# minjiyoon/MMGL

Hardware: AMD Instinct MI355X
Metric: train samples/sec (OPT-1.3B flamingo, 16 neighbors) (higher is better)
Workload: dtype bf16; 1 GPU; opt-1.3b context=all neighbor_mode=embedding peft=flamingo, 11+5 neighbors x 4 tokens, T=512+128, roberta-base + clip-vit-base-patch16 frozen encoders, full train step (fwd+bwd+exchange+AdamW); per_gpu_batch=64, global_batch=64, seq_len=640, neighbor_keys=64, trainable_params=216736520, parallelism=dp1

## Files before the change

include/mmgl_hip.h:

```cpp
#ifndef MMGL_HIP_H
#define MMGL_HIP_H

#include <stddef.h>
#include <stdint.h>

#ifdef __cplusplus
extern "C" {
#endif

enum { MMGL_F32 = 0, MMGL_BF16 = 1 };
enum { MMGL_OK = 0, MMGL_ERR_INVALID = 1, MMGL_ERR_UNSUPPORTED = 2, MMGL_ERR_HIP = 3 };
enum { MMGL_ACT_NONE = 0, MMGL_ACT_RELU = 1 };

const char* mmgl_last_error(void);
int mmgl_version(void);

int mmgl_xattn_fwd(const void* q, const void* k, const void* v, const uint8_t* key_valid,
                   void* out, float* lse, int B, int H, int T, int S, int D, int dtype, void* stream);

size_t mmgl_xattn_bwd_workspace(int B, int H, int T, int S, int D);
int mmgl_xattn_bwd(const void* dout, const void* q, const void* k, const void* v, const float* lse,
                   const uint8_t* key_valid, void* dq, void* dk, void* dv,
                   void* workspace, size_t workspace_bytes,
                   int B, int H, int T, int S, int D, int dtype, void* stream);
// ... 51 lines not shown
size_t mmgl_norm_bwd_workspace(int rows, int cols);
int mmgl_layernorm_bwd(const void* dy, const void* x, const void* gamma, const float* mean, const float* rstd,
                       void* dx, float* dgamma, float* dbeta, void* workspace, size_t workspace_bytes,
                       int rows, int cols, int dtype, void* stream);

int mmgl_rmsnorm_fwd(const void* x, const void* gamma, void* y, float* rstd,
                     int rows, int cols, float eps, int dtype, void* stream);
int mmgl_rmsnorm_bwd(const void* dy, const void* x, const void* gamma, const float* rstd,
                     void* dx, float* dgamma, void* workspace, size_t workspace_bytes,
                     int rows, int cols, int dtype, void* stream);

int mmgl_add_rmsnorm_fwd(const void* x, const void* res, const void* gamma, void* sum_out, void* y, float* rstd,
                         int rows, int cols, float eps, int dtype, void* stream);
int mmgl_add_rmsnorm_bwd(const void* dy, const void* dsum, const void* sum, const void* gamma, const float* rstd,
                         void* dres, float* dgamma, void* workspace, size_t workspace_bytes,
                         int rows, int cols, int dtype, void* stream);

int mmgl_gated_residual_fwd(const void* residual, const void* x, const float* gate, void* y,
                            size_t n, float p_drop, uint64_t seed, int dtype, void* stream);
size_t mmgl_gated_residual_bwd_workspace(size_t n);
int mmgl_gated_residual_bwd(const void* dy, const void* x, const float* gate, void* dx, float* dgate,
                            void* workspace, size_t workspace_bytes,
                            size_t n, float p_drop, uint64_t seed, int dtype, void* stream);

int mmgl_linear_fwd(const void* x, const void* W, const void* bias, void* y,
                    int M, int N, int K, int act, float out_scale, int dtype, void* stream);
size_t mmgl_linear_bwd_workspace(int M, int N, int K, int act, int dtype);
int mmgl_linear_bwd(const void* dy, const void* y, const void* x, const void* W, void* dx, void* dW, void* dbias,
                    void* workspace, size_t workspace_bytes, int M, int N, int K, int act, float out_scale,
                    int accumulate, int mask_dx, int dtype, void* stream);

int mmgl_lora_linear_fwd(const void* x, const void* W, const void* bias, const void* A, const void* Bm,
                         void* y, void* xa, int M, int N, int K, int r, float scale, int dtype, void* stream);
size_t mmgl_lora_linear_bwd_workspace(int M, int N, int K, int r, int dtype);
int mmgl_lora_linear_bwd(const void* dy, const void* x, const void* xa, const void* W, const void* A,
                         const void* Bm, void* dx, void* dA, void* dB, void* dyb, void* workspace,
                         size_t workspace_bytes, int M, int N, int K, int r, float scale, int accumulate,
                         int dtype, void* stream);

int mmgl_neighbor_interleave_fwd(const void* text_emb, const void* vis_emb, const int64_t* text_loc,
                                 const int64_t* img_loc, const int64_t* text_pos, const int64_t* img_pos,
                                 void* out_emb, uint8_t* out_valid, int B, int Nt, int Ni, int n_tok, int d,
                                 int dtype, void* stream);
int mmgl_neighbor_interleave_bwd(const void* d_out_emb, const int64_t* text_loc, const int64_t* img_loc,
                                 void* d_text_emb, void* d_vis_emb, int B, int Nt, int Ni, int n_tok, int d,
                                 int dtype, void* stream);

int mmgl_cross_entropy_fwd(const void* logits, const int64_t* labels, float* row_lse, float* row_loss,
                           float* loss_sum, float* count, int rows, int V, int64_t ignore_index, int dtype,
                           void* stream);
int mmgl_cross_entropy_bwd(const void* logits, const int64_t* labels, const float* row_lse,
                           const float* count, const float* dloss, void* dlogits,
                           int rows, int V, int64_t ignore_index, int dtype, void* stream);

int mmgl_position_ids(const int64_t* attention_mask, int64_t* pos, int B, int T, void* stream);

int mmgl_adamw_step(void* param, float* master, const void* grad, float* exp_avg, float* exp_avg_sq, size_t n,
                    float lr, float beta1, float beta2, float eps, float weight_decay, int step,
                    float grad_scale, int dtype, void* stream);

size_t mmgl_adafactor_workspace(const int64_t* segs, int n, int64_t* table_out);
int mmgl_adafactor_step(void* param, float* master, const void* grad, float* state, const int64_t* table, const int64_t* table_host,
                        int n, void* workspace, size_t workspace_bytes, float lr, float eps1, float clip_threshold, double decay_rate,
                        float weight_decay, int step, float grad_scale, int dtype, void* stream);

int mmgl_gemm_nt_fast(int M, int N, int K, int ldx, int ldw, int ldy, int dtype);
size_t mmgl_gemm_nt_workspace(int M, int N, int K, int ldx, int ldw, int ldy, int dtype);
int mmgl_gemm_nt(const void* x, int ldx, const void* W, int ldw, const void* bias, const void* residual, const void* zmask,
                 void* y, int ldy, int M, int N, int K, int act, float out_scale, void* workspace, size_t workspace_bytes,
                 int dtype, void* stream);
int mmgl_relu_bwd(const void* dy, const void* y, void* out, size_t n, int dtype, void* stream);
int mmgl_gemm_nt_rowk(const void* x, int ldx, const void* W, int ldw, void* y, int ldy, int M, int N, int K, int K_short,
                      int m_full, int dtype, void* stream);
int mmgl_gemm_nt_rowk_item(int G, int n_long, int n_short, int q, int wg, int it);
int mmgl_gemm_set_tile_counter(void* counter);
void* mmgl_gemm_get_tile_counter(void);
size_t mmgl_gemm_nt_relu_bits_bytes(int M, int N, int K, int ldx, int ldw, int ldy, int dtype);
int mmgl_gemm_nt_relu_bits(const void* x, int ldx, const void* W, int ldw, const void* bias, void* y, int ldy, void* bits_out,
                           int M, int N, int K, float out_scale, int dtype, void* stream);
int mmgl_gemm_nt_masked(const void* x, int ldx, const void* W, int ldw, const void* bits_in, void* y, int ldy, int M, int N, int K,
                        float out_scale, int dtype, void* stream);

int mmgl_rope_inplace(void* buf, const float* cos_sin, size_t rows, int T, int H, int D, int ld, int nblk, int backward,
                      int dtype, void* stream);
int mmgl_rope(const void* src, void* dst, const float* cos_sin, size_t rows, int T, int H, int D, int ld, int nblk, int nall,
              int backward, int dtype, void* stream);
int mmgl_swiglu_fwd(const void* gate_up, void* y, size_t M, int F, int dtype, void* stream);
int mmgl_swiglu_bwd(const void* dy, const void* gate_up, void* dgate_up, size_t M, int F, int dtype, void* stream);

int mmgl_encattn_fwd(const void* q, const void* k, const void* v, const int32_t* cu_seqlens, void* out, int nseq,
                     int H, int D, int ld_in, int ld_out, int max_len, int q_rows, int dtype, void* stream);
int mmgl_add_layernorm_fwd(const void* x, const void* res, const void* gamma, const void* beta, void* sum_out,
                           void* y, float* mean, float* rstd, int rows, int cols, float eps, float p_drop, uint64_t seed,
                           int dtype, void* stream);
int mmgl_add_layernorm_bwd(const void* dy, const void* dsum, const void* sum, const void* gamma, const float* mean,
                           const float* rstd, void* dres, void* dx, float* dgamma, float* dbeta, void* workspace,
                           size_t workspace_bytes, int rows, int cols, float p_drop, uint64_t seed, int dtype,
                           void* stream);
int mmgl_layernorm_tiles_fwd(const void* x, const void* gamma, const void* beta, void* y, void* yc, const int32_t* rowmap,
                             float* mean, float* rstd, int rows, int cols, int crows, float eps, int dtype, void* stream);
int mmgl_add_layernorm_tiles_fwd(const void* x, const void* res, const void* gamma, const void* beta, void* sum_out, void* y,
                                 void* yc, const int32_t* rowmap, float* mean, float* rstd, int rows, int cols, int crows,
                                 float eps, float p_drop, uint64_t seed, int dtype, void* stream);
int mmgl_add_layernorm_rows_bwd(const void* dy, const int32_t* dy_rows, const void* dsum, const void* sum, const void* gamma,
                                const float* mean, const float* rstd, void* dres, void* dx, float* dgamma, float* dbeta,
                                void* workspace, size_t workspace_bytes, int rows, int cols, float p_drop, uint64_t seed,
// ... 95 lines not shown
```

mmgl_amd/_lib.py:

```python
import ctypes
import os

import torch

_HERE = os.path.dirname(os.path.abspath(__file__))
LIB_PATH = os.environ.get("MMGL_LIB_PATH") or os.path.join(_HERE, "libmmgl_hip.so")

ABI_VERSION = 110
F32, BF16 = 0, 1
ACT_NONE, ACT_RELU = 0, 1
_ERR_INVALID, _ERR_UNSUPPORTED, _ERR_HIP = 1, 2, 3

c_void_p, c_int, c_float, c_size_t, c_u64, c_i64 = (ctypes.c_void_p, ctypes.c_int, ctypes.c_float, ctypes.c_size_t,
                                                    ctypes.c_uint64, ctypes.c_int64)
P, I, F, Z, U, L = c_void_p, c_int, c_float, c_size_t, c_u64, c_i64
D = ctypes.c_double

SIGNATURES = {
    "mmgl_last_error": (ctypes.c_char_p, []),
    "mmgl_version": (I, []),
    "mmgl_xattn_fwd": (I, [P, P, P, P, P, P, I, I, I, I, I, I, P]),
    "mmgl_xattn_bwd_workspace": (Z, [I, I, I, I, I]),
    "mmgl_xattn_bwd": (I, [P, P, P, P, P, P, P, P, P, P, Z, I, I, I, I, I, I, P]),
    "mmgl_selfattn_fwd": (I, [P, P, P, P, P, P, I, I, I, I, I, I, P]),
    "mmgl_selfattn_bwd_workspace": (Z, [I, I, I]),
    "mmgl_selfattn_bwd": (I, [P, P, P, P, P, P, P, P, P, P, P, Z, I, I, I, I, I, I, I, P]),
    "mmgl_selfattn_prefix_fwd": (I, [P, P, P, P, P, P, I, I, I, I, I, I, I, I, P]),
    "mmgl_selfattn_prefix_bwd": (I, [P, P, P, P, P, P, P, P, P, P, P, Z, I, I, I, I, I, I, I, I, I, I, P]),
    "mmgl_selfattn_tiles_fwd": (I, [P, P, P, P, P, P, P, I, I, I, I, I, I, I, I, P]),
    "mmgl_selfattn_tiles_bwd": (I, [P, P, P, P, P, P, P, P, P, P, P, P, Z, I, I, I, I, I, I, I, I, I, I, P]),
    "mmgl_selfattn_tiles_rows_bwd": (I, [P, P, P, P, P, P, P, P, P, P, P, P, P, Z, I, I, I, I, I, I, I, I, I, I, I, P]),
    "mmgl_selfattn_gqa_fwd": (I, [P, P, P, P, P, P, I, I, I, I, I, I, I, I, P]),
    "mmgl_selfattn_gqa_bwd_workspace": (Z, [I, I, I, I, I, I]),
    "mmgl_selfattn_gqa_bwd": (I, [P, P, P, P, P, P, P, P, P, P, P, Z, I, I, I, I, I, I, I, I, I, I, P]),
    "mmgl_attn_general_fwd": (I, [P, P, P, P, P, P, P, P, I, I, I, I, I, I, F, U, I, P]),
    "mmgl_attn_general_bwd_workspace": (Z, [I, I, I]),
    "mmgl_attn_general_bwd": (I, [P, P, P, P, P, P, P, P, P, P, P, Z, I, I, I, I, I, I, F, U, I, P]),
    "mmgl_attn_dropout_mask": (I, [P, I, I, I, I, F, U, P]),
    "mmgl_attn_relbias_fwd": (I, [P, P, P, P, P, P, P, P, I, I, I, I, I, I, I, I, I, F, U, I, P]),
    "mmgl_attn_relbias_bwd_workspace": (Z, [I, I, I, I]),
    "mmgl_attn_relbias_bwd": (I, [P, P, P, P, P, P, P, P, P, P, P, P, P, P, Z, I, I, I, I, I, I, I, I, I, F, U, I, P]),
    "mmgl_layernorm_fwd": (I, [P, P, P, P, P, P, I, I, F, I, P]),
    "mmgl_norm_bwd_workspace": (Z, [I, I]),
    "mmgl_layernorm_bwd": (I, [P, P, P, P, P, P, P, P, P, Z, I, I, I, P]),
    "mmgl_rmsnorm_fwd": (I, [P, P, P, P, I, I, F, I, P]),
    "mmgl_rmsnorm_bwd": (I, [P, P, P, P, P, P, P, Z, I, I, I, P]),
    "mmgl_add_rmsnorm_fwd": (I, [P, P, P, P, P, P, I, I, F, I, P]),
    "mmgl_add_rmsnorm_bwd": (I, [P, P, P, P, P, P, P, P, Z, I, I, I, P]),
    "mmgl_gated_residual_fwd": (I, [P, P, P, P, Z, F, U, I, P]),
    "mmgl_gated_residual_bwd_workspace": (Z, [Z]),
    "mmgl_gated_residual_bwd": (I, [P, P, P, P, P, P, Z, Z, F, U, I, P]),
    "mmgl_linear_fwd": (I, [P, P, P, P, I, I, I, I, F, I, P]),
    "mmgl_linear_bwd_workspace": (Z, [I, I, I, I, I]),
    "mmgl_linear_bwd": (I, [P, P, P, P, P, P, P, P, Z, I, I, I, I, F, I, I, I, P]),
    "mmgl_lora_linear_fwd": (I, [P, P, P, P, P, P, P, I, I, I, I, F, I, P]),
    "mmgl_lora_linear_bwd_workspace": (Z, [I, I, I, I, I]),
    "mmgl_lora_linear_bwd": (I, [P, P, P, P, P, P, P, P, P, P, P, Z, I, I, I, I, F, I, I, P]),
    "mmgl_neighbor_interleave_fwd": (I, [P, P, P, P, P, P, P, P, I, I, I, I, I, I, P]),
    "mmgl_neighbor_interleave_bwd": (I, [P, P, P, P, P, I, I, I, I, I, I, P]),
    "mmgl_cross_entropy_fwd": (I, [P, P, P, P, P, P, I, I, L, I, P]),
    "mmgl_cross_entropy_bwd": (I, [P, P, P, P, P, P, I, I, L, I, P]),
    "mmgl_position_ids": (I, [P, P, I, I, P]),
    "mmgl_adamw_step": (I, [P, P, P, P, P, Z, F, F, F, F, F, I, F, I, P]),
    "mmgl_encattn_fwd": (I, [P, P, P, P, P, I, I, I, I, I, I, I, I, P]),
    "mmgl_add_layernorm_fwd": (I, [P, P, P, P, P, P, P, P, I, I, F, F, U, I, P]),
    "mmgl_add_layernorm_bwd": (I, [P, P, P, P, P, P, P, P, P, P, P, Z, I, I, F, U, I, P]),
    "mmgl_layernorm_tiles_fwd": (I, [P, P, P, P, P, P, P, P, I, I, I, F, I, P]),
    "mmgl_add_layernorm_tiles_fwd": (I, [P, P, P, P, P, P, P, P, P, P, I, I, I, F, F, U, I, P]),
    "mmgl_activation_fwd": (I, [P, P, Z, I, I, P]),
    "mmgl_scale": (I, [P, P, P, Z, I, P]),
    "mmgl_gemm_nt_fast": (I, [I, I, I, I, I, I, I]),
    "mmgl_gemm_nt_workspace": (Z, [I, I, I, I, I, I, I]),
    "mmgl_gemm_nt_relu_bits_bytes": (Z, [I, I, I, I, I, I, I]),
    "mmgl_gemm_nt_relu_bits": (I, [P, I, P, I, P, P, I, P, I, I, I, F, I, P]),
    "mmgl_gemm_nt_masked": (I, [P, I, P, I, P, P, I, I, I, I, F, I, P]),
    "mmgl_gemm_nt": (I, [P, I, P, I, P, P, P, P, I, I, I, I, I, F, P, Z, I, P]),
    "mmgl_gemm_nt_rowk": (I, [P, I, P, I, P, I, I, I, I, I, I, I, P]),
    "mmgl_gemm_nt_rowk_item": (I, [I, I, I, I, I, I]),
    "mmgl_add_layernorm_rows_bwd": (I, [P, P, P, P, P, P, P, P, P, P, P, P, Z, I, I, F, U, I, P]),
    "mmgl_relu_bwd": (I, [P, P, P, Z, I, P]),
    "mmgl_gemm_set_tile_counter": (I, [P]),
    "mmgl_gemm_get_tile_counter": (P, []),
    "mmgl_rope_inplace": (I, [P, P, Z, I, I, I, I, I, I, I, P]),
    "mmgl_rope": (I, [P, P, P, Z, I, I, I, I, I, I, I, I, P]),
    "mmgl_swiglu_fwd": (I, [P, P, Z, I, I, P]),
    "mmgl_swiglu_bwd": (I, [P, P, P, Z, I, I, P]),
    "mmgl_comm_unique_id": (I, [P]),
    "mmgl_comm_init": (I, [I, I, P, ctypes.POINTER(ctypes.c_void_p)]),
    "mmgl_allreduce_sum": (I, [P, P, Z, I, P]),
    "mmgl_allgather": (I, [P, P, P, Z, I, P]),
    "mmgl_broadcast": (I, [P, P, Z, I, I, P]),
    "mmgl_comm_destroy": (I, [P]),
    "mmgl_gemm_skinny": (I, [P, I, P, I, P, P, P, I, I, I, I, I, F, I, P]),
    "mmgl_attn_decode_fwd": (I, [P, I, P, P, I, Z, P, I, P, I, I, I, I, I, P]),
    "mmgl_gemm_skinny_lora": (I, [P, I, P, I, P, P, P, I, P, I, P, I, I, F, P, I, I, I, I, F, I, P]),
    "mmgl_attn_decode_gqa_fwd": (I, [P, I, P, P, I, Z, P, I, P, I, I, I, I, I, I, P]),
    "mmgl_rope_kv_append": (I, [P, I, P, P, Z, I, I, I, I, I, P]),
    "mmgl_attn_decode_beam_fwd": (I, [P, I, P, P, I, Z, P, I, P, P, I, Z, P, I, P, I, I, I, I, I, I, I, P]),
    "mmgl_beam_topk_workspace": (Z, [I, I, I]),
    "mmgl_beam_topk": (I, [P, Z, P, P, P, P, Z, I, I, I, I, I, P]),
    "mmgl_beam_advance": (I, [P, P, P, P, P, P, P, I, P, P, P, P, P, P, P, P, P, I, I, I, I, I, I, I, F, P]),
    "mmgl_sample_tokens": (I, [P, Z, P, P, L, P, P, I, I, I, F, I, F, I, L, I, P]),
    "mmgl_logits_process": (I, [P, Z, P, Z, P, Z, I, I, P, I, I, I, F, I, I, P]),
    "mmgl_guidance_logits": (I, [P, Z, I, I, F, I, P]),
    "mmgl_attn_decode_block_fwd": (I, [P, I, P, P, I, P, P, I, Z, I, P, I, P, P, I, I, I, I, I, P]),
    "mmgl_lookup_accept": (I, [P, Z, I, P, P, P, P, Z, P, Z, P, P, P, P, I, I, I, I, I, I, L, L, I, I, I, P]),
    "mmgl_rope_kv_append_block": (I, [P, I, P, I, P, I, Z, I, P, I, I, I, I, I, I, P]),
    "mmgl_attn_decode_gqa_block_fwd": (I, [P, I, P, P, I, Z, I, P, I, P, P, I, I, I, I, I, I, P]),
    "mmgl_contrastive_chunk": (I, []),
    "mmgl_contrastive_workspace": (Z, [I, I, I]),
    "mmgl_contrastive_select": (I, [P, Z, P, Z, Z, P, Z, I, P, P, Z, F, I, I, P, Z, P, Z, P, L, L, P, P, P, P, P, P, Z, I, I, I, I, I, P]),
    "mmgl_kv_quantize": (I, [P, P, I, Z, P, I, Z, P, I, Z, I, I, I, I, I, P]),
    "mmgl_attn_decode_q8_fwd": (I, [P, I, P, P, I, P, P, I, Z, P, P, I, Z, I, P, I, P, I, I, I, I, I, P]),
    "mmgl_attn_decode_gqa_q8_fwd": (I, [P, I, P, P, I, P, P, I, Z, P, P, I, Z, I, P, I, P, I, I, I, I, I, I, P]),
# ... 45 lines not shown


def ptr(t):
    return None if t is None else ctypes.c_void_p(t.data_ptr())


def ptr_off(t, nbytes):
    return ctypes.c_void_p(t.data_ptr() + int(nbytes))


_raw_stream = getattr(torch._C, "_cuda_getCurrentRawStream", None)
_raw_device = getattr(torch._C, "_cuda_getDevice", None)


def stream_ptr():
    if _raw_stream is not None and _raw_device is not None:
        return ctypes.c_void_p(_raw_stream(_raw_device()))
    return ctypes.c_void_p(torch.cuda.current_stream().cuda_stream)


def require_cuda(*ts):
    for t in ts:
        if t is not None and not t.is_cuda:
            raise RuntimeError("mmgl_amd ops run on the GPU only (tensor is on %s); there is no CPU path" % t.device)


class KernelTimer:
    enabled = False
    only = None
    records = []
    by_tag = bool(os.environ.get("MMGL_KERNEL_TAGS"))

    @classmethod
    def reset(cls):
        cls.records = []

    @classmethod
    def summary(cls):
        torch.cuda.synchronize()
        out = {}
        for name, s, e, work in cls.records:
            if cls.by_tag and "tag" in work:
                name = f"{name}[{work['tag']}]"
            d = out.setdefault(name, dict(calls=0, ms_total=0.0, bytes=0.0, flops=0.0))
            d["calls"] += 1
            d["ms_total"] += s.elapsed_time(e)
            d["bytes"] += work.get("bytes", 0.0)
            d["flops"] += work.get("flops", 0.0)
        for d in out.values():
            d["ms_avg"] = d["ms_total"] / d["calls"]
        return out


def call(name: str, work, *args):
    fn = getattr(lib(), name)
    if KernelTimer.enabled and (KernelTimer.only is None or name in KernelTimer.only):
        s = torch.cuda.Event(enable_timing=True)
        e = torch.cuda.Event(enable_timing=True)
        s.record()
        rc = fn(*args)
        e.record()
        KernelTimer.records.append((name, s, e, work() if callable(work) else (work or {})))
    else:
        rc = fn(*args)
    check(rc, name)
```

mmgl_amd/csrc/elementwise.hip:

```cpp
#include "common.h"

namespace {

template <typename T> struct Vec {
    static constexpr int N = 16 / sizeof(T);
    typedef T type __attribute__((ext_vector_type(16 / sizeof(T))));
};

__device__ __forceinline__ float block_sum(float v, float* red) {
    v = wave_sum(v);
    __syncthreads();
    if ((threadIdx.x & 63) == 0) red[threadIdx.x >> 6] = v;
    __syncthreads();
    return red[0] + red[1] + red[2] + red[3];
}
__device__ __forceinline__ float block_max(float v, float* red) {
    v = wave_max(v);
    __syncthreads();
    if ((threadIdx.x & 63) == 0) red[threadIdx.x >> 6] = v;
    __syncthreads();
    return fmaxf(fmaxf(red[0], red[1]), fmaxf(red[2], red[3]));
}

inline int stream_blocks(size_t nvec) {
// ... 211 lines not shown

__global__ __launch_bounds__(256) void ce_finish_kernel(const float* __restrict__ row_loss, const int64_t* __restrict__ labels,
                                                        int rows, int V_, int64_t ignore, float* __restrict__ loss_sum,
                                                        float* __restrict__ count) {
    __shared__ float red[4];
    float a = 0.f, c = 0.f;
    for (int i = threadIdx.x; i < rows; i += 256) {
        const int64_t lab = labels[i];
        if (!(lab == ignore || lab < 0 || lab >= V_)) { a += row_loss[i]; c += 1.f; }
    }
    const float sa = block_sum(a, red);
    const float sc = block_sum(c, red);
    if (threadIdx.x == 0) { *loss_sum = sa; *count = sc; }
}

template <typename T>
__global__ __launch_bounds__(256) void ce_bwd_kernel(const T* __restrict__ logits, const int64_t* __restrict__ labels,
                                                     const float* __restrict__ row_lse, const float* __restrict__ count,
                                                     const float* __restrict__ dloss, T* __restrict__ dlogits, int V_,
                                                     int64_t ignore) {
    typedef typename Vec<T>::type V;
    constexpr int VN = Vec<T>::N;
    const int row = blockIdx.x;
    const T* x = logits + (size_t)row * V_;
    T* dx = dlogits + (size_t)row * V_;
    const int64_t lab = labels[row];
    const bool ign = (lab == ignore || lab < 0 || lab >= V_);
    const float scale = ign ? 0.f : (*dloss) / fmaxf(*count, 1.f);
    const float lse = row_lse[row];
    const int nvec = (((size_t)V_ * sizeof(T)) % 16 == 0) ? V_ / VN : 0;
    auto grad = [&](int i, const V& v) __attribute__((always_inline)) {
        V o;
#pragma unroll
        for (int j = 0; j < VN; ++j) {
            float g = __expf((float)v[j] - lse);
            if (i * VN + j == lab) g -= 1.f;
            o[j] = (T)(g * scale);
        }
        ((V*)dx)[i] = o;
    };
    int i = threadIdx.x;
    for (; i + 768 < nvec; i += 1024) {
        const V v0 = ((const V*)x)[i], v1 = ((const V*)x)[i + 256], v2 = ((const V*)x)[i + 512], v3 = ((const V*)x)[i + 768];
        grad(i, v0);
        grad(i + 256, v1);
        grad(i + 512, v2);
        grad(i + 768, v3);
    }
    for (; i < nvec; i += 256) grad(i, ((const V*)x)[i]);
    for (int i = nvec * VN + threadIdx.x; i < V_; i += 256) {
        float g = __expf((float)x[i] - lse);
        if (i == lab) g -= 1.f;
        dx[i] = (T)(g * scale);
    }
}

__global__ __launch_bounds__(64) void position_ids_kernel(const int64_t* __restrict__ mask, int64_t* __restrict__ pos, int T_) {
    const int b = blockIdx.x, lane = threadIdx.x;
    int64_t carry = 0;
    for (int t0 = 0; t0 < T_; t0 += 64) {
        const int t = t0 + lane;
        const int64_t m = t < T_ ? mask[(size_t)b * T_ + t] : 0;
        int64_t v = m;
#pragma unroll
        for (int o = 1; o < 64; o <<= 1) {
            const int64_t u = __shfl_up(v, o);
            if (lane >= o) v += u;
        }
        if (t < T_) pos[(size_t)b * T_ + t] = (carry + v) * m - 1 + 2;
        carry += __shfl(v, 63);
    }
}

template <typename T>
__global__ __launch_bounds__(256) void adamw_kernel(T* __restrict__ param, float* __restrict__ master,
                                                    const T* __restrict__ grad, float* __restrict__ m,
                                                    float* __restrict__ v, size_t n, float lr, float b1, float b2,
                                                    float eps, float wd, float bc1, float bc2s, float gscale) {
    for (size_t i = (size_t)blockIdx.x * 256 + threadIdx.x; i < n; i += (size_t)gridDim.x * 256) {
        const float g = (float)grad[i] * gscale;
        float p = master ? master[i] : (float)param[i];
        p *= 1.f - lr * wd;
        const float mi = b1 * m[i] + (1.f - b1) * g;
        const float vi = b2 * v[i] + (1.f - b2) * g * g;
        m[i] = mi;
        v[i] = vi;
        p -= (lr / bc1) * mi / (sqrtf(vi) / bc2s + eps);
        if (master) master[i] = p;
        param[i] = (T)p;
    }
}

}

#define BY_DTYPE(CALL_BF16, CALL_F32, who)                        \
    do {                                                          \
        if (dtype == MMGL_BF16) { CALL_BF16; }                    \
        else if (dtype == MMGL_F32) { CALL_F32; }                 \
        else MMGL_FAIL(MMGL_ERR_INVALID, "%s: bad dtype %d", who, dtype); \
    } while (0)

extern "C" int mmgl_gated_residual_fwd(const void* residual, const void* x, const float* gate, void* y, size_t n,
                                       float p_drop, uint64_t seed, int dtype, void* stream) {
    MMGL_CHECK_ARG(residual && x && y, "mmgl_gated_residual_fwd: null pointer");
    MMGL_CHECK_ARG(p_drop >= 0.f && p_drop < 1.f, "mmgl_gated_residual_fwd: dropout p=%g outside [0,1)", p_drop);
    if (n == 0) return MMGL_OK;
// ... 55 lines not shown
}

extern "C" int mmgl_neighbor_interleave_bwd(const void* d_out_emb, const int64_t* text_loc, const int64_t* img_loc,
                                            void* d_text_emb, void* d_vis_emb, int B, int Nt, int Ni, int n_tok, int d,
                                            int dtype, void* stream) {
    MMGL_CHECK_ARG(B > 0 && Nt >= 0 && Ni >= 0 && Nt + Ni > 0 && n_tok > 0 && d > 0, "mmgl_neighbor_interleave_bwd: bad sizes");
    MMGL_CHECK_ARG(d_out_emb && (Nt == 0 || (d_text_emb && text_loc)) && (Ni == 0 || (d_vis_emb && img_loc)),
                   "mmgl_neighbor_interleave_bwd: null pointer");
    MMGL_CHECK_ARG(n_tok <= 256, "mmgl_neighbor_interleave_bwd: n_tok > 256");
    MMGL_CHECK_ARG(dtype == MMGL_BF16 || dtype == MMGL_F32, "mmgl_neighbor_interleave_bwd: bad dtype %d", dtype);
    const size_t esz = dtype == MMGL_BF16 ? 2 : 4;
    if (((size_t)n_tok * d * esz) % 16) MMGL_FAIL(MMGL_ERR_UNSUPPORTED, "mmgl_neighbor_interleave_bwd: n_tok*d must cover whole 16-byte chunks");
    hipStream_t st = (hipStream_t)stream;
    const int N = Nt + Ni;
    BY_DTYPE(hipLaunchKernelGGL(interleave_bwd_kernel<bf16>, dim3(B * N), dim3(256), 0, st, (const bf16*)d_out_emb, text_loc,
                                img_loc, (bf16*)d_text_emb, (bf16*)d_vis_emb, Nt, Ni, n_tok, d),
             hipLaunchKernelGGL(interleave_bwd_kernel<float>, dim3(B * N), dim3(256), 0, st, (const float*)d_out_emb, text_loc,
                                img_loc, (float*)d_text_emb, (float*)d_vis_emb, Nt, Ni, n_tok, d),
             "mmgl_neighbor_interleave_bwd");
    MMGL_CHECK_LAUNCH("mmgl_neighbor_interleave_bwd");
    return MMGL_OK;
}

extern "C" int mmgl_cross_entropy_fwd(const void* logits, const int64_t* labels, float* row_lse, float* row_loss,
                                      float* loss_sum, float* count, int rows, int V, int64_t ignore_index, int dtype,
                                      void* stream) {
    MMGL_CHECK_ARG(logits && labels && row_lse && row_loss && loss_sum && count, "mmgl_cross_entropy_fwd: null pointer");
    MMGL_CHECK_ARG(rows > 0 && V > 0, "mmgl_cross_entropy_fwd: bad sizes");
    hipStream_t st = (hipStream_t)stream;
    BY_DTYPE(hipLaunchKernelGGL(ce_fwd_kernel<bf16>, dim3(rows), dim3(256), 0, st, (const bf16*)logits, labels, row_lse,
                                row_loss, V, ignore_index),
             hipLaunchKernelGGL(ce_fwd_kernel<float>, dim3(rows), dim3(256), 0, st, (const float*)logits, labels, row_lse,
                                row_loss, V, ignore_index),
             "mmgl_cross_entropy_fwd");
    hipLaunchKernelGGL(ce_finish_kernel, dim3(1), dim3(256), 0, st, row_loss, labels, rows, V, ignore_index, loss_sum, count);
    MMGL_CHECK_LAUNCH("mmgl_cross_entropy_fwd");
    return MMGL_OK;
}

extern "C" int mmgl_cross_entropy_bwd(const void* logits, const int64_t* labels, const float* row_lse, const float* count,
                                      const float* dloss, void* dlogits, int rows, int V, int64_t ignore_index, int dtype,
                                      void* stream) {
    MMGL_CHECK_ARG(logits && labels && row_lse && count && dloss && dlogits, "mmgl_cross_entropy_bwd: null pointer");
    hipStream_t st = (hipStream_t)stream;
    BY_DTYPE(hipLaunchKernelGGL(ce_bwd_kernel<bf16>, dim3(rows), dim3(256), 0, st, (const bf16*)logits, labels, row_lse, count,
                                dloss, (bf16*)dlogits, V, ignore_index),
             hipLaunchKernelGGL(ce_bwd_kernel<float>, dim3(rows), dim3(256), 0, st, (const float*)logits, labels, row_lse,
                                count, dloss, (float*)dlogits, V, ignore_index),
             "mmgl_cross_entropy_bwd");
    MMGL_CHECK_LAUNCH("mmgl_cross_entropy_bwd");
    return MMGL_OK;
}

extern "C" int mmgl_position_ids(const int64_t* attention_mask, int64_t* pos, int B, int T, void* stream) {
    MMGL_CHECK_ARG(attention_mask && pos && B > 0 && T > 0, "mmgl_position_ids: bad arguments");
    hipLaunchKernelGGL(position_ids_kernel, dim3(B), dim3(64), 0, (hipStream_t)stream, attention_mask, pos, T);
    MMGL_CHECK_LAUNCH("mmgl_position_ids");
    return MMGL_OK;
}

extern "C" int mmgl_adamw_step(void* param, float* master, const void* grad, float* exp_avg, float* exp_avg_sq, size_t n,
                               float lr, float beta1, float beta2, float eps, float weight_decay, int step,
                               float grad_scale, int dtype, void* stream) {
    MMGL_CHECK_ARG(param && grad && exp_avg && exp_avg_sq && step >= 1, "mmgl_adamw_step: bad arguments");
    if (n == 0) return MMGL_OK;
    const float bc1 = (float)(1.0 - pow((double)beta1, (double)step));
    const float bc2s = (float)sqrt(1.0 - pow((double)beta2, (double)step));
    hipStream_t st = (hipStream_t)stream;
    const int blocks = stream_blocks(n);
    BY_DTYPE(hipLaunchKernelGGL(adamw_kernel<bf16>, dim3(blocks), dim3(256), 0, st, (bf16*)param, master, (const bf16*)grad,
                                exp_avg, exp_avg_sq, n, lr, beta1, beta2, eps, weight_decay, bc1, bc2s, grad_scale),
             hipLaunchKernelGGL(adamw_kernel<float>, dim3(blocks), dim3(256), 0, st, (float*)param, master, (const float*)grad,
                                exp_avg, exp_avg_sq, n, lr, beta1, beta2, eps, weight_decay, bc1, bc2s, grad_scale),
             "mmgl_adamw_step");
    MMGL_CHECK_LAUNCH("mmgl_adamw_step");
    return MMGL_OK;
}

template <typename T> static int act_launch(const void* x, void* y, size_t n, int act, hipStream_t st) {
    const int blocks = stream_blocks(n / (16 / sizeof(T)));
    switch (act) {
        case 1: hipLaunchKernelGGL((act_kernel<T, 1>), dim3(blocks), dim3(256), 0, st, (const T*)x, (T*)y, n); break;
        case 2: hipLaunchKernelGGL((act_kernel<T, 2>), dim3(blocks), dim3(256), 0, st, (const T*)x, (T*)y, n); break;
        case 3: hipLaunchKernelGGL((act_kernel<T, 3>), dim3(blocks), dim3(256), 0, st, (const T*)x, (T*)y, n); break;
        default: hipLaunchKernelGGL((act_kernel<T, 4>), dim3(blocks), dim3(256), 0, st, (const T*)x, (T*)y, n); break;
    }
    MMGL_CHECK_LAUNCH("mmgl_activation_fwd");
    return MMGL_OK;
}

extern "C" int mmgl_activation_fwd(const void* x, void* y, size_t n, int act, int dtype, void* stream) {
    MMGL_CHECK_ARG(x && y, "mmgl_activation_fwd: null pointer");
    MMGL_CHECK_ARG(act >= 1 && act <= 4, "mmgl_activation_fwd: act %d not in {1 relu, 2 gelu, 3 quick_gelu, 4 gelu_tanh}", act);
    if (n == 0) return MMGL_OK;
    hipStream_t st = (hipStream_t)stream;
    if (dtype == MMGL_BF16) return act_launch<bf16>(x, y, n, act, st);
    if (dtype == MMGL_F32) return act_launch<float>(x, y, n, act, st);
    MMGL_FAIL(MMGL_ERR_INVALID, "mmgl_activation_fwd: bad dtype %d", dtype);
}

extern "C" int mmgl_scale(const void* x, const float* scale, void* y, size_t n, int dtype, void* stream) {
    MMGL_CHECK_ARG(x && y && scale, "mmgl_scale: null pointer");
    if (n == 0) return MMGL_OK;
    hipStream_t st = (hipStream_t)stream;
    if (dtype == MMGL_BF16) hipLaunchKernelGGL(scale_kernel<bf16>, dim3(stream_blocks(n / 8)), dim3(256), 0, st, (const bf16*)x, scale, (bf16*)y, n);
    else if (dtype == MMGL_F32) hipLaunchKernelGGL(scale_kernel<float>, dim3(stream_blocks(n / 4)), dim3(256), 0, st, (const float*)x, scale, (float*)y, n);
// ... 5 lines not shown
```

mmgl_amd/model/modelling_cross_attention.py:

```python
import math
import os
from typing import List, Optional, Tuple, Union

import torch
import torch.nn as nn
import torch.nn.functional as F
from transformers import (AutoConfig, AutoModelForCausalLM, CLIPTextModel, CLIPVisionModel, PretrainedConfig,
                          RobertaModel)
from transformers.activations import ACT2FN
from transformers.modeling_outputs import BaseModelOutputWithPast, CausalLMOutputWithPast

from .. import ops
from .decode_cache import BeamState, DecodeCache, LookupState, StepCodes
from .encoders import ClipTextEncoder, PackedTextEncoder, PackedVisionEncoder
from .generation import beam_loop, check_prompt, contrastive_loop, decode_loop, lookup_loop, make_select
from .sampling import (check_contrastive, check_guidance, check_kv_cache, check_lookup, check_processors, check_sampling,
                       check_weight_dtype)

CROSS_MODES = ("cross_attention", "embedding")


def uses_cross_attention(neighbor_mode: str, peft_type: str = "flamingo") -> bool:
    return neighbor_mode == "cross_attention" or (neighbor_mode == "embedding" and peft_type == "flamingo")

# ... 743 lines not shown
        return h

    def _verify_step(self, cache):
        lookup = cache.lookup
        if lookup is None or cache.beam is not None or cache.next_pos is None:
            raise ValueError("a verify step needs a prefilled DecodeCache with a LookupState (cache.lookup) and no BeamState")
        ops.require_cuda(cache.mask)
        with torch.no_grad():
            return self._decode_rows(self.embed_tokens(lookup.block.view(-1)), lookup.positions.view(-1), cache)


class MPTModel(MPTPreTrainedModel):
    def __init__(self, config: MPTConfig):
        super().__init__(config)
        self.decoder = MPTDecoder(config)

    def get_input_embeddings(self):
        return self.decoder.embed_tokens

    def set_input_embeddings(self, value):
        self.decoder.embed_tokens = value

    def get_decoder(self):
        return self.decoder

    def forward(self, *args, **kwargs):
        return self.decoder(*args, **kwargs)


def reset_peft_parameters(model):
    for n, p in model.named_parameters():
        if "lora_A" in n:
            nn.init.kaiming_uniform_(p, a=math.sqrt(5))
        if "lora_B" in n:
            nn.init.zeros_(p)


def mark_only_peft_as_trainable(model):
    for p in model.parameters():
        p.requires_grad = False
    for m in model.modules():
        if isinstance(m, MPTDecoderLayer) and m.cross_attention:
            for p in m.parameters():
                p.requires_grad = True


def lm_head_loss_and_logits(module, lm_head, hidden, next_labels, return_logits=None, logits_slice=None):
    frozen = type(lm_head) is nn.Linear and not lm_head.weight.requires_grad and lm_head.bias is None
    lanes = 16 // hidden.element_size()
    aligned = lm_head.weight.shape[0] % lanes == 0 and lm_head.weight.shape[1] % lanes == 0
    opted_out = return_logits is False or (return_logits is None and logits_slice is not None)
    fuse = next_labels is not None and frozen and hidden.is_cuda and opted_out and aligned
    if fuse:
        loss = ops.lm_head_cross_entropy(hidden, lm_head.weight, next_labels)
        logits = None
        if logits_slice is not None:
            with torch.no_grad():
                logits = _lin(lm_head, hidden.detach()[:, logits_slice].contiguous())
        return loss, logits
    logits = _lin(lm_head, hidden)
    loss = None
    if next_labels is not None:
        loss = ops.cross_entropy(logits.view(-1, logits.shape[-1]), next_labels.view(-1))
    if logits_slice is not None:
        logits = logits[:, logits_slice]
    return loss, logits


class MPTForCausalLM(MPTPreTrainedModel):
    _tied_weights_keys = ["lm_head.weight"]

    def __init__(self, config):
        super().__init__(config)
        self.model = MPTModel(config)
        self.lm_head = nn.Linear(config.word_embed_proj_dim, config.vocab_size, bias=False)
        self.lm_head.apply(self._init_weights)
        self.lm_head.weight = self.model.decoder.embed_tokens.weight
        if config.peft_type != "none":
            reset_peft_parameters(self.model)
            mark_only_peft_as_trainable(self.model)

    def get_input_embeddings(self):
        return self.model.decoder.embed_tokens

    def set_input_embeddings(self, value):
        self.model.decoder.embed_tokens = value

    def get_output_embeddings(self):
        return self.lm_head

    def set_output_embeddings(self, new_embeddings):
        self.lm_head = new_embeddings

    def set_decoder(self, decoder):
        self.model.decoder = decoder

    def get_decoder(self):
        return self.model.decoder

    def forward(self, input_ids=None, attention_mask=None, head_mask=None, past_key_values=None, inputs_embeds=None,
                labels=None, neighbor_embeds=None, neighbor_attention_mask=None, use_cache=None, output_attentions=None,
                output_hidden_states=None, return_dict=None, first_key_valid=False, return_logits=None, logits_slice=None,
                cache_capacity=None, key_tiles=None, kv_cache_dtype=None):
        return_dict = True if return_dict is None else return_dict
        outputs = self.model.decoder(input_ids=input_ids, attention_mask=attention_mask, head_mask=head_mask,
                                     past_key_values=past_key_values, inputs_embeds=inputs_embeds,
                                     neighbor_embeds=neighbor_embeds, neighbor_attention_mask=neighbor_attention_mask,
                                     use_cache=use_cache, output_attentions=output_attentions,
                                     output_hidden_states=output_hidden_states, return_dict=True, first_key_valid=first_key_valid,
# ... 457 lines not shown
```

mmgl_amd/ops.py:

```python
import math
import os
import weakref

import torch
import torch.nn.functional as F

from . import _lib
from ._lib import dtype_code, lib, ptr, ptr_off, require_cuda, stream_ptr


def _dropout(p_drop, training, seed):
    p = float(p_drop) if training else 0.0
    if p > 0.0 and seed is None:
        seed = int(torch.randint(0, 2 ** 62, (1,)).item())
    return p, int(seed or 0)


def _check_mask(key_valid, shape):
    if key_valid.shape != shape:
        raise ValueError(f"Attention mask should be of size {tuple(shape)}, but is {tuple(key_valid.shape)}")


def _key_valid(key_valid):
    if key_valid.dtype != torch.uint8:
# ... 998 lines not shown
        ctx.mark_non_differentiable(valid)
        return out, valid

    @staticmethod
    def backward(ctx, dout, _dvalid):
        tl, il = ctx.saved_tensors
        B, Nt, Ni, n_tok, d = ctx.dims
        dout = dout.contiguous()
        dtext = torch.empty(B, Nt, n_tok, d, dtype=dout.dtype, device=dout.device)
        dvis = torch.empty(B, Ni, n_tok, d, dtype=dout.dtype, device=dout.device) if Ni else None
        _lib.call("mmgl_neighbor_interleave_bwd", None, ptr(dout), ptr(tl), ptr(il), ptr(dtext), ptr(dvis), B, Nt, Ni, n_tok, d,
                                                 dtype_code(dout), stream_ptr())
        return dtext, dvis, None, None, None, None


def neighbor_interleave(text_emb, vis_emb, text_loc, img_loc, text_pos, img_pos):
    if vis_emb is not None and vis_emb.shape[2:] != text_emb.shape[2:]:
        raise ValueError("n_text_tokens must equal n_visual_tokens for the interleaved layout (reference :1083-1098)")
    return _Interleave.apply(text_emb, vis_emb, text_loc, img_loc, text_pos, img_pos)


class _CrossEntropy(torch.autograd.Function):
    @staticmethod
    def forward(ctx, logits, labels, ignore_index):
        require_cuda(logits, labels)
        rows, V = logits.shape
        logits = logits.contiguous()
        labels = labels.contiguous()
        dev = logits.device
        row_lse = torch.empty(rows, dtype=torch.float32, device=dev)
        row_loss = torch.empty(rows, dtype=torch.float32, device=dev)
        sums = torch.empty(2, dtype=torch.float32, device=dev)
        _lib.call("mmgl_cross_entropy_fwd", dict(bytes=1.0 * rows * V * logits.element_size()), ptr(logits), ptr(labels), ptr(row_lse), ptr(row_loss), ptr(sums[0:1]), ptr(sums[1:2]),
                                           rows, V, ignore_index, dtype_code(logits), stream_ptr())
        ctx.save_for_backward(logits, labels, row_lse, sums)
        ctx.ignore = ignore_index
        return sums[0] / sums[1]

    @staticmethod
    def backward(ctx, dloss):
        logits, labels, row_lse, sums = ctx.saved_tensors
        rows, V = logits.shape
        dl = dloss.detach().to(torch.float32).reshape(1).contiguous()
        dlogits = torch.empty_like(logits)
        _lib.call("mmgl_cross_entropy_bwd", dict(bytes=2.0 * rows * V * logits.element_size()), ptr(logits), ptr(labels), ptr(row_lse), ptr(sums[1:2]), ptr(dl), ptr(dlogits), rows, V,
                                           ctx.ignore, dtype_code(logits), stream_ptr())
        return dlogits, None, None


def cross_entropy(logits, labels, ignore_index=-100):
    return _CrossEntropy.apply(logits, labels, int(ignore_index))


class _LMHeadCrossEntropy(torch.autograd.Function):

    @staticmethod
    def forward(ctx, hidden, weight, labels, ignore_index, chunk_rows):
        require_cuda(hidden, weight, labels)
        V, d = weight.shape
        h2 = hidden.reshape(-1, d)
        if not h2.is_contiguous():
            h2 = h2.contiguous()
        M = h2.shape[0]
        lab = labels.reshape(-1).contiguous()
        dev = h2.device
        w = weight if weight.dtype == h2.dtype else weight.to(h2.dtype)
        count = (lab != ignore_index).sum().to(torch.float32).reshape(1)
        one = torch.ones(1, dtype=torch.float32, device=dev)
        loss_sum = torch.zeros(1, dtype=torch.float32, device=dev)
        dh = torch.empty_like(h2)
        chunk = min(M, int(chunk_rows))
        scratch = torch.empty(chunk, V, dtype=h2.dtype, device=dev)
        row_lse = torch.empty(chunk, dtype=torch.float32, device=dev)
        row_loss = torch.empty(chunk, dtype=torch.float32, device=dev)
        part = torch.empty(2, dtype=torch.float32, device=dev)
        code = dtype_code(h2)
        es = h2.element_size()
        for r0 in range(0, M, chunk):
            r1 = min(M, r0 + chunk)
            n = r1 - r0
            lg = scratch[:n]
            gemm_nt(h2[r0:r1], w.contiguous(), out=lg)
            _lib.call("mmgl_cross_entropy_fwd", dict(bytes=1.0 * n * V * es), ptr(lg), ptr(lab[r0:r1]), ptr(row_lse), ptr(row_loss), ptr(part[0:1]),
                      ptr(part[1:2]), n, V, ignore_index, code, stream_ptr())
            loss_sum += part[0:1]
            _lib.call("mmgl_cross_entropy_bwd", dict(bytes=2.0 * n * V * es), ptr(lg), ptr(lab[r0:r1]), ptr(row_lse), ptr(count), ptr(one), ptr(lg), n, V,
                      ignore_index, code, stream_ptr())
            frozen_dgrad(lg, weight, out=dh[r0:r1])
        ctx.save_for_backward(dh)
        ctx.shape = hidden.shape
        return (loss_sum / count.clamp_min(1.0)).reshape(())

    @staticmethod
    def backward(ctx, dloss):
        (dh,) = ctx.saved_tensors
        s = dloss.detach().to(torch.float32).reshape(1).contiguous()
        out = torch.empty_like(dh)
        _lib.call("mmgl_scale", dict(bytes=2.0 * dh.numel() * dh.element_size()), ptr(dh), ptr(s), ptr(out), dh.numel(), dtype_code(dh),
                  stream_ptr())
        return out.view(ctx.shape), None, None, None, None


def lm_head_cross_entropy(hidden, weight, labels, ignore_index=-100, chunk_rows=8192):
    if weight.requires_grad:
        raise ValueError("lm_head_cross_entropy: the head must be frozen (use lm_head + cross_entropy for a trainable head)")
    if hidden.shape[:-1] != labels.shape or hidden.shape[-1] != weight.shape[1]:
        raise ValueError(f"lm_head_cross_entropy: shapes hidden{tuple(hidden.shape)} weight{tuple(weight.shape)} labels{tuple(labels.shape)}")
    return _LMHeadCrossEntropy.apply(hidden, weight, labels, int(ignore_index), int(chunk_rows))


def position_ids(attention_mask):
    require_cuda(attention_mask)
    m = attention_mask.to(torch.int64).contiguous()
    out = torch.empty_like(m)
    _lib.call("mmgl_position_ids", None, ptr(m), ptr(out), m.shape[0], m.shape[1], stream_ptr())
    return out


def adamw_step_(param, master, grad, exp_avg, exp_avg_sq, lr, beta1, beta2, eps, weight_decay, step, grad_scale=1.0):
    require_cuda(param, grad)
    _lib.call("mmgl_adamw_step", None, ptr(param), ptr(master), ptr(grad), ptr(exp_avg), ptr(exp_avg_sq), param.numel(), lr, beta1, beta2,
                                eps, weight_decay, step, grad_scale, dtype_code(param), stream_ptr())


class AdafactorTable:

    def __init__(self, segments):
        import ctypes
        self.shapes, self.offsets, self.state_offsets = [], [], []
        rows, st = [], 0
        for off, shape in segments:
            shape = tuple(int(s) for s in shape)
            if not 1 <= len(shape) <= 2:
                raise ValueError(f"fused Adafactor takes 1-D and 2-D tensors, got shape {shape}: transformers factors a tensor of more "
                                 "dimensions over its last two with the leading ones as a batch, which this kernel does not do")
            R, C = (shape[0], 0) if len(shape) == 1 else shape
            if C == 0 and len(shape) == 2 or R == 0:
                raise ValueError(f"fused Adafactor: empty tensor of shape {shape}")
            self.shapes.append(shape), self.offsets.append(int(off)), self.state_offsets.append(st)
            rows += [int(off), R, C, st]
            st += (R + C + 31) // 32 * 32
        self.n, self.state_numel = len(self.shapes), st
        if not self.n:
            raise ValueError("fused Adafactor: no tensors")
        segs = (ctypes.c_int64 * len(rows))(*rows)
        self.host = (ctypes.c_int64 * (8 * (self.n + 1)))()
        self.workspace_bytes = lib().mmgl_adafactor_workspace(segs, self.n, self.host)
        if not self.workspace_bytes:
            raise ValueError(lib().mmgl_last_error().decode("utf-8", "replace"))
        self.n_tiles, self.n_folds = int(self.host[8 * self.n + 4]), int(self.host[8 * self.n + 5])
        self.device = self.workspace = None

    def to(self, device):
        self.device = torch.tensor(list(self.host), dtype=torch.int64).to(device)
        self.workspace = torch.empty(self.workspace_bytes, dtype=torch.uint8, device=device)
        return self


def adafactor_step_(param, master, grad, state, table, lr, step, grad_scale=1.0, weight_decay=0.0, eps1=1e-30, clip_threshold=1.0,
                    decay_rate=-0.8):
    require_cuda(param, grad, state, table.device, table.workspace)
# ... 1126 lines not shown
```

Baseline: 289.5 samples/s.

## Fuse cross-entropy forward and backward into one register-resident chunk kernel

Adds a bf16 kernel that loads each logits row into registers once, computes the online log-sum-exp and loss, then writes the gradient in place. This replaces the separate forward and backward cross-entropy passes, which read the large logits chunk twice. The kernel can also write out requested logits positions while the row is loaded, so the extra LM-head GEMM for logits_slice is skipped. It keeps unsupported dtypes and shapes on a fallback path, at the cost of heavy register pressure and more complex Python autograd plumbing.

```diff
diff --git a/include/mmgl_hip.h b/include/mmgl_hip.h
--- a/include/mmgl_hip.h
+++ b/include/mmgl_hip.h
@@ -127,6 +127,9 @@
 int mmgl_cross_entropy_bwd(const void* logits, const int64_t* labels, const float* row_lse,
                            const float* count, const float* dloss, void* dlogits,
                            int rows, int V, int64_t ignore_index, int dtype, void* stream);
+int mmgl_cross_entropy_chunk(void* logits, const int64_t* labels, float* row_lse, float* row_loss, float* loss_sum,
+                             float* count_part, const float* count, const float* dloss, const int* slice_rows,
+                             void* slice_out, int slice_n, int rows, int V, int64_t ignore_index, int dtype, void* stream);
 
 int mmgl_position_ids(const int64_t* attention_mask, int64_t* pos, int B, int T, void* stream);
 
diff --git a/mmgl_amd/_lib.py b/mmgl_amd/_lib.py
--- a/mmgl_amd/_lib.py
+++ b/mmgl_amd/_lib.py
@@ -60,6 +60,7 @@
     "mmgl_neighbor_interleave_bwd": (I, [P, P, P, P, P, I, I, I, I, I, I, P]),
     "mmgl_cross_entropy_fwd": (I, [P, P, P, P, P, P, I, I, L, I, P]),
     "mmgl_cross_entropy_bwd": (I, [P, P, P, P, P, P, I, I, L, I, P]),
+    "mmgl_cross_entropy_chunk": (I, [P, P, P, P, P, P, P, P, P, P, I, I, I, L, I, P]),
     "mmgl_position_ids": (I, [P, P, I, I, P]),
     "mmgl_adamw_step": (I, [P, P, P, P, P, Z, F, F, F, F, F, I, F, I, P]),
     "mmgl_encattn_fwd": (I, [P, P, P, P, P, I, I, I, I, I, I, I, I, P]),
@@ -211,7 +212,7 @@
         return out
 
 
-def call(name: str, work, *args):
+def _invoke(name, work, args):
     fn = getattr(lib(), name)
     if KernelTimer.enabled and (KernelTimer.only is None or name in KernelTimer.only):
         s = torch.cuda.Event(enable_timing=True)
@@ -220,6 +221,17 @@
         rc = fn(*args)
         e.record()
         KernelTimer.records.append((name, s, e, work() if callable(work) else (work or {})))
-    else:
-        rc = fn(*args)
+        return rc
+    return fn(*args)
+
+
+def call(name: str, work, *args):
+    check(_invoke(name, work, args), name)
+
+
+def call_if_supported(name: str, work, *args) -> bool:
+    rc = _invoke(name, work, args)
+    if rc == _ERR_UNSUPPORTED:
+        return False
     check(rc, name)
+    return True
diff --git a/mmgl_amd/csrc/elementwise.hip b/mmgl_amd/csrc/elementwise.hip
--- a/mmgl_amd/csrc/elementwise.hip
+++ b/mmgl_amd/csrc/elementwise.hip
@@ -287,6 +287,89 @@
         float g = __expf((float)x[i] - lse);
         if (i == lab) g -= 1.f;
         dx[i] = (T)(g * scale);
+    }
+}
+
+__device__ __forceinline__ float mul_then_add(float a, float b, float c) {
+#pragma clang fp contract(off)
+    const float p = a * b;
+    return p + c;
+}
+
+template <int NV>
+__global__ __launch_bounds__(256, NV <= 25 ? 4 : 3) void ce_chunk_kernel(bf16* logits, const int64_t* __restrict__ labels,
+                                                                         float* __restrict__ row_lse, float* __restrict__ row_loss,
+                                                                         const float* __restrict__ count, const float* __restrict__ dloss,
+                                                                         const int* __restrict__ slice_rows, bf16* __restrict__ slice_out,
+                                                                         int slice_n, int V_, int64_t ignore) {
+    typedef bf16 T;
+    typedef typename Vec<T>::type V;
+    constexpr int VN = Vec<T>::N;
+    __shared__ float red[4];
+    __shared__ float lse_sh;
+    const int row = blockIdx.x, tid = threadIdx.x;
+    T* x = logits + (size_t)row * V_;
+    const int nvec = V_ / VN;
+    V v[NV];
+#pragma unroll
+    for (int k = 0; k < NV; ++k) v[k] = tid < nvec - k * 256 ? ((const V*)(x + (size_t)k * 256 * VN))[tid] : vzero<V>();
+    float m = -INFINITY, s = 0.f;
+    auto fold = [&](const V& v, bool fused) __attribute__((always_inline)) {
+        float lm = (float)v[0];
+#pragma unroll
+        for (int j = 1; j < VN; ++j) lm = fmaxf(lm, (float)v[j]);
+        const float nm = fmaxf(m, lm);
+        const float sh = nm == -INFINITY ? 0.f : nm;
+        float acc = 0.f;
+#pragma unroll
+        for (int j = 0; j < VN; ++j) acc += __expf((float)v[j] - sh);
+        const float e = __expf(m - sh);
+        s = fused ? __builtin_fmaf(s, e, acc) : mul_then_add(s, e, acc);
+        m = nm;
+    };
+#pragma unroll
+    for (int k = 0; k < NV; ++k)
+        if (tid < nvec - k * 256) fold(v[k], k % 2 == 1 || tid >= nvec - 768 - 1024 * (k / 4));
+    const int srow = slice_rows ? slice_rows[row] : -1;
+    if (srow >= 0 && srow < slice_n) {
+        T* so = slice_out + (size_t)srow * V_;
+#pragma unroll
+        for (int k = 0; k < NV; ++k)
+            if (tid < nvec - k * 256) ((V*)(so + (size_t)k * 256 * VN))[tid] = v[k];
+    }
+    const float gm = block_max(m, red);
+    const float gs = block_sum(m == -INFINITY ? 0.f : s * __expf(m - gm), red);
+    const int64_t lab = labels[row];
+    const bool ign = (lab == ignore || lab < 0 || lab >= V_);
+    if (tid == 0) {
+        const float lse = gm + logf(gs);
+        row_lse[row] = lse;
+        row_loss[row] = ign ? 0.f : lse - (float)x[lab];
+        lse_sh = lse;
+    }
+    __syncthreads();
+    const float lse = lse_sh;
+    const float scale = ign ? 0.f : (*dloss) / fmaxf(*count, 1.f);
+    typedef uint32_t W __attribute__((ext_vector_type(4)));
+#pragma unroll
+    for (int k = 0; k < NV; ++k) {
+        W w = __builtin_bit_cast(W, v[k]);
+        asm volatile("" : "+v"(w.x), "+v"(w.y), "+v"(w.z), "+v"(w.w));
+        v[k] = __builtin_bit_cast(V, w);
+    }
+#pragma unroll
+    for (int k = 0; k < NV; ++k) {
+        if (tid < nvec - k * 256) {
+            const int64_t labk = lab - (int64_t)k * 256 * VN;
+            V o;
+#pragma unroll
+            for (int j = 0; j < VN; ++j) {
+                float g = __expf((float)v[k][j] - lse);
+                if (tid * VN + j == labk) g -= 1.f;
+                o[j] = (T)(g * scale);
+            }
+            ((V*)(x + (size_t)k * 256 * VN))[tid] = o;
+        }
     }
 }
 
@@ -448,6 +531,35 @@
     return MMGL_OK;
 }
 
+extern "C" int mmgl_cross_entropy_chunk(void* logits, const int64_t* labels, float* row_lse, float* row_loss, float* loss_sum,
+                                        float* count_part, const float* count, const float* dloss, const int* slice_rows,
+                                        void* slice_out, int slice_n, int rows, int V, int64_t ignore_index, int dtype,
+                                        void* stream) {
+    MMGL_CHECK_ARG(logits && labels && row_lse && row_loss && loss_sum && count_part && count && dloss,
+                   "mmgl_cross_entropy_chunk: null pointer");
+    MMGL_CHECK_ARG(rows > 0 && V > 0, "mmgl_cross_entropy_chunk: bad sizes");
+    MMGL_CHECK_ARG(dtype == MMGL_BF16 || dtype == MMGL_F32, "mmgl_cross_entropy_chunk: bad dtype %d", dtype);
+    MMGL_CHECK_ARG(!slice_rows || (slice_out && slice_n > 0), "mmgl_cross_entropy_chunk: slice_rows without slice_out");
+    if (dtype != MMGL_BF16) MMGL_FAIL(MMGL_ERR_UNSUPPORTED, "mmgl_cross_entropy_chunk: bf16 only (fp32: mmgl_cross_entropy_fwd + _bwd)");
+    if (V % 8 || V > 256 * 32 * 8)
+        MMGL_FAIL(MMGL_ERR_UNSUPPORTED, "mmgl_cross_entropy_chunk: V = %d is no multiple of 8 or exceeds 65536 (mmgl_cross_entropy_fwd + _bwd)", V);
+    if ((uintptr_t)logits % 16 || (uintptr_t)slice_out % 16)
+        MMGL_FAIL(MMGL_ERR_UNSUPPORTED, "mmgl_cross_entropy_chunk: logits and slice_out must be 16-byte aligned");
+    hipStream_t st = (hipStream_t)stream;
+    const int per_thread = (V / 8 + 255) / 256;
+#define MMGL_CE_CHUNK(NV)                                                                                                               \
+    hipLaunchKernelGGL(ce_chunk_kernel<NV>, dim3(rows), dim3(256), 0, st, (bf16*)logits, labels, row_lse, row_loss, count, dloss,       \
+                       slice_rows, (bf16*)slice_out, slice_n, V, ignore_index)
+    if (per_thread <= 4) MMGL_CE_CHUNK(4);
+    else if (per_thread <= 16) MMGL_CE_CHUNK(16);
+    else if (per_thread <= 25) MMGL_CE_CHUNK(25);
+    else MMGL_CE_CHUNK(32);
+#undef MMGL_CE_CHUNK
+    hipLaunchKernelGGL(ce_finish_kernel, dim3(1), dim3(256), 0, st, row_loss, labels, rows, V, ignore_index, loss_sum, count_part);
+    MMGL_CHECK_LAUNCH("mmgl_cross_entropy_chunk");
+    return MMGL_OK;
+}
+
 extern "C" int mmgl_position_ids(const int64_t* attention_mask, int64_t* pos, int B, int T, void* stream) {
     MMGL_CHECK_ARG(attention_mask && pos && B > 0 && T > 0, "mmgl_position_ids: bad arguments");
     hipLaunchKernelGGL(position_ids_kernel, dim3(B), dim3(64), 0, (hipStream_t)stream, attention_mask, pos, T);
diff --git a/mmgl_amd/model/modelling_cross_attention.py b/mmgl_amd/model/modelling_cross_attention.py
--- a/mmgl_amd/model/modelling_cross_attention.py
+++ b/mmgl_amd/model/modelling_cross_attention.py
@@ -819,9 +819,10 @@
     opted_out = return_logits is False or (return_logits is None and logits_slice is not None)
     fuse = next_labels is not None and frozen and hidden.is_cuda and opted_out and aligned
     if fuse:
-        loss = ops.lm_head_cross_entropy(hidden, lm_head.weight, next_labels)
-        logits = None
-        if logits_slice is not None:
+        if logits_slice is None:
+            return ops.lm_head_cross_entropy(hidden, lm_head.weight, next_labels), None
+        loss, logits = ops.lm_head_cross_entropy(hidden, lm_head.weight, next_labels, logits_slice=logits_slice)
+        if logits is None:
             with torch.no_grad():
                 logits = _lin(lm_head, hidden.detach()[:, logits_slice].contiguous())
         return loss, logits
diff --git a/mmgl_amd/ops.py b/mmgl_amd/ops.py
--- a/mmgl_amd/ops.py
+++ b/mmgl_amd/ops.py
@@ -1074,10 +1074,27 @@
     return _CrossEntropy.apply(logits, labels, int(ignore_index))
 
 
+_SLICE_ROWS = {}
+
+
+def _slice_rows_table(B, T, positions, device):
+    key = (B, T, positions, device)
+    tab = _SLICE_ROWS.get(key)
+    if tab is None:
+        if len(_SLICE_ROWS) >= 16:
+            _SLICE_ROWS.clear()
+        one = torch.full((T,), -1, dtype=torch.int64)
+        one[list(positions)] = torch.arange(len(positions))
+        full = one[None, :] + torch.arange(B)[:, None] * len(positions)
+        full[:, one < 0] = -1
+        tab = _SLICE_ROWS[key] = full.reshape(-1).to(torch.int32).to(device)
+    return tab
+
+
 class _LMHeadCrossEntropy(torch.autograd.Function):
 
     @staticmethod
-    def forward(ctx, hidden, weight, labels, ignore_index, chunk_rows):
+    def forward(ctx, hidden, weight, labels, ignore_index, chunk_rows, slice_pos=None, _pair=False):
         require_cuda(hidden, weight, labels)
         V, d = weight.shape
         h2 = hidden.reshape(-1, d)
@@ -1098,37 +1115,61 @@
         part = torch.empty(2, dtype=torch.float32, device=dev)
         code = dtype_code(h2)
         es = h2.element_size()
+        one_pass = not _pair
+        table = sl = None
+        if slice_pos is not None and one_pass:
+            B, T = hidden.shape[:2]
+            sl = torch.empty(B, len(slice_pos), V, dtype=h2.dtype, device=dev)
+            table = _slice_rows_table(B, T, slice_pos, dev) if slice_pos else None
         for r0 in range(0, M, chunk):
             r1 = min(M, r0 + chunk)
             n = r1 - r0
             lg = scratch[:n]
             gemm_nt(h2[r0:r1], w.contiguous(), out=lg)
-            _lib.call("mmgl_cross_entropy_fwd", dict(bytes=1.0 * n * V * es), ptr(lg), ptr(lab[r0:r1]), ptr(row_lse), ptr(row_loss), ptr(part[0:1]),
-                      ptr(part[1:2]), n, V, ignore_index, code, stream_ptr())
-            loss_sum += part[0:1]
-            _lib.call("mmgl_cross_entropy_bwd", dict(bytes=2.0 * n * V * es), ptr(lg), ptr(lab[r0:r1]), ptr(row_lse), ptr(count), ptr(one), ptr(lg), n, V,
-                      ignore_index, code, stream_ptr())
+            if one_pass:
+                one_pass = _lib.call_if_supported("mmgl_cross_entropy_chunk", dict(bytes=2.0 * n * V * es), ptr(lg), ptr(lab[r0:r1]), ptr(row_lse),
+                                                  ptr(row_loss), ptr(part[0:1]), ptr(part[1:2]), ptr(count), ptr(one),
+                                                  *((None, None, 0) if table is None else (ptr(table[r0:r1]), ptr(sl), sl.shape[0] * sl.shape[1])),
+                                                  n, V, ignore_index, code, stream_ptr())
+            if one_pass:
+                loss_sum += part[0:1]
+            else:
+                _lib.call("mmgl_cross_entropy_fwd", dict(bytes=1.0 * n * V * es), ptr(lg), ptr(lab[r0:r1]), ptr(row_lse), ptr(row_loss), ptr(part[0:1]),
+                          ptr(part[1:2]), n, V, ignore_index, code, stream_ptr())
+                loss_sum += part[0:1]
+                _lib.call("mmgl_cross_entropy_bwd", dict(bytes=2.0 * n * V * es), ptr(lg), ptr(lab[r0:r1]), ptr(row_lse), ptr(count), ptr(one), ptr(lg), n, V,
+                          ignore_index, code, stream_ptr())
             frozen_dgrad(lg, weight, out=dh[r0:r1])
         ctx.save_for_backward(dh)
         ctx.shape = hidden.shape
-        return (loss_sum / count.clamp_min(1.0)).reshape(())
-
-    @staticmethod
-    def backward(ctx, dloss):
+        loss = (loss_sum / count.clamp_min(1.0)).reshape(())
+        if not one_pass:
+            sl = None
+        if sl is not None:
+            ctx.mark_non_differentiable(sl)
+        return loss, sl
+
+    @staticmethod
+    def backward(ctx, dloss, _dslice=None):
         (dh,) = ctx.saved_tensors
         s = dloss.detach().to(torch.float32).reshape(1).contiguous()
         out = torch.empty_like(dh)
         _lib.call("mmgl_scale", dict(bytes=2.0 * dh.numel() * dh.element_size()), ptr(dh), ptr(s), ptr(out), dh.numel(), dtype_code(dh),
                   stream_ptr())
-        return out.view(ctx.shape), None, None, None, None
-
-
-def lm_head_cross_entropy(hidden, weight, labels, ignore_index=-100, chunk_rows=8192):
+        return out.view(ctx.shape), None, None, None, None, None, None
+
+
+def lm_head_cross_entropy(hidden, weight, labels, ignore_index=-100, chunk_rows=8192, logits_slice=None, _pair=False):
     if weight.requires_grad:
         raise ValueError("lm_head_cross_entropy: the head must be frozen (use lm_head + cross_entropy for a trainable head)")
     if hidden.shape[:-1] != labels.shape or hidden.shape[-1] != weight.shape[1]:
         raise ValueError(f"lm_head_cross_entropy: shapes hidden{tuple(hidden.shape)} weight{tuple(weight.shape)} labels{tuple(labels.shape)}")
-    return _LMHeadCrossEntropy.apply(hidden, weight, labels, int(ignore_index), int(chunk_rows))
+    if logits_slice is None:
+        return _LMHeadCrossEntropy.apply(hidden, weight, labels, int(ignore_index), int(chunk_rows), None, bool(_pair))[0]
+    if hidden.dim() != 3:
+        raise ValueError(f"lm_head_cross_entropy: logits_slice needs hidden [B, T, d], got {tuple(hidden.shape)}")
+    pos = tuple(range(hidden.shape[1])[logits_slice])
+    return _LMHeadCrossEntropy.apply(hidden, weight, labels, int(ignore_index), int(chunk_rows), pos, bool(_pair))
 
 
 def position_ids(attention_mask):
```

After: 282.0 samples/s. -2.6%, worse.
